# SJLeo/GCC

Hardware: AMD Instinct MI355X
Metric: training images/sec at 256x256 (pix2pix GCC) (higher is better)
Workload: dtype bf16; 1 GPU; Pix2Pix cityscapes 256x256 GCC distill+darts iteration (optimize_parameters + optimizer_netD_arch), student ngf32 / masked PatchGAN ndf128, teacher ngf64 / ndf128, filter_cfgs=None (no pretrained checkpoint to prune); batch_per_gpu=16, global_batch=16, image=256x256, parallelism=dp1, dropout=on (counter RNG; the oracle / golden iterations run --no_dropout)

## Files before the change

### gcc_amd/_lib.py

```python
import ctypes as C
import os

_HERE = os.path.dirname(os.path.abspath(__file__))
LIB_PATH = os.environ.get('GCC_HIP_LIB') or os.path.join(_HERE, 'libgcc_hip.so')

ACT_NONE, ACT_LRELU, ACT_RELU, ACT_TANH = 0, 1, 2, 3
GCC_HIP_ABI = 605
WGRAD_GROUP_MAX = 32
CHANSUM_GROUP_MAX = 24
SPECTRAL_GROUP_MAX = 8
CHANSUM_SMALL_MAX_PIXELS = 16384


class GccError(RuntimeError):
    pass


class conv_plan_t(C.Structure):
    _fields_ = [(n, C.c_int) for n in ('tile_families', 'big_min', 'big_nk', 'pair', 'halo_hc', 'wgrad_wgs_big', 'wgrad_wgs')]


PLAN_FIELDS = tuple(n for n, _ in conv_plan_t._fields_)


# ... 206 lines not shown
    'gcc_conv_eval_ex_workspace': (_Z, [C.POINTER(conv_t), _I]),
    'gcc_conv_eval_ex_route': (_I, [C.POINTER(conv_t), _I, _Z]),
    'gcc_conv_eval_f32': (_I, [C.POINTER(conv_t), _P, _P, _P, C.POINTER(eval_f32_epilogue_t), _P]),
    'gcc_conv_eval_f32_route': (_I, [C.POINTER(conv_t), _I]),
    'gcc_conv_eval_f32_kp': (_I, [_I, _I, _I]),
    'gcc_conv_eval_f32_ex': (_I, [C.POINTER(conv_t), _I, _I, _P, _P, _P, C.POINTER(eval_f32_epilogue_t), _P]),
    'gcc_conv_eval_f32_ex_route': (_I, [C.POINTER(conv_t), _I, _I, _I]),
    'gcc_conv_eval_f32_act': (_I, [C.POINTER(conv_t), _I, _I, _P, _P, _P, C.POINTER(eval_f32_act_epilogue_t), _P]),
    'gcc_conv_eval_f32_act_route': (_I, [C.POINTER(conv_t), _I, _I, _I, _I]),
    'gcc_conv_eval_f32_unet': (_I, [C.POINTER(conv_t), _I, _P, _P, _P, C.POINTER(eval_f32_unet_epilogue_t), _P]),
    'gcc_conv_eval_f32_unet_route': (_I, [C.POINTER(conv_t), _I]),
    'gcc_conv_eval_f32_unet_kp': (_I, [_I, _I]),
    'gcc_conv_eval_f32_resnet': (_I, [C.POINTER(conv_t), _I, _P, _P, _P, C.POINTER(eval_f32_resnet_epilogue_t), _P]),
    'gcc_conv_eval_f32_resnet_route': (_I, [C.POINTER(conv_t), _I]),
    'gcc_conv_eval_f32_resnet_kp': (_I, [_I, _I, _I]),
    'gcc_dwconv3x3_reflect_f32': (_I, [_P, _I, _P, _I, _P, _P, _I, _I, _I, _I, _P, _Z, _P]),
    'gcc_inorm_f32_workspace': (_Z, [_I, _I, C.c_longlong]),
    'gcc_inorm_stats_f32': (_I, [_P, _I, _I, _I, _I, _I, _P, _Z, _P]),
    'gcc_inorm_apply_f32': (_I, [_P, _I, _P, _I, _P, _I, _I, _I, _I, _I, _I, _F, _P, _Z, _P]),
    'gcc_nhwc_f32_to_nchw_f32': (_I, [_P, _P, _I, _I, _I, _I, _I, _I, _P]),
    'gcc_nchw_f32_to_nhwc_f32': (_I, [_P, _P, _I, _I, _I, _I, _I, _I, _I, _P]),
    'gcc_image_to_u8': (_I, [_P, _I, _I, _Z, _P, _P]),
    'gcc_image_to_u8_f32': (_I, [_P, _I, _I, _Z, _P, _P]),
    'gcc_dw_inorm_fwd': (_I, [C.POINTER(dw_inorm_t), _P]),
    'gcc_dw_inorm_route': (_I, [C.POINTER(dw_inorm_t)]),
    'gcc_dw_inorm_plan': (_I, [C.POINTER(dw_inorm_t), _I]),
    'gcc_conv_bn_act': (_I, [C.POINTER(conv_t), _I, _P, _P, _P, C.POINTER(bn_t), C.POINTER(bnact_t), _P, _I, _I, _P, _I, _I, _P, _Z, _P]),
    'gcc_conv_bn_act_plan': (_I, [C.POINTER(conv_t), _I, C.POINTER(bn_t), _I]),
    'gcc_bnact_bwd_workspace': (_Z, [_I, _Z]),
    'gcc_bnact_bwd': (_I, [C.POINTER(bnact_bwd_t), _P, _I, _I, _P, _I, _I, _P, _I, _I, _P, _I, _I, _P, _I, _I,
                           _I, _Z, _P, _Z, _P]),
    'gcc_bnact_bwd_ex': (_I, [C.POINTER(bnact_bwd_t), _I, _F, _P, _I, _I, _P, _I, _I, _P, _I, _I, _P, _I, _I, _P,
                              _I, _I, _I, _Z, _P, _Z, _P]),
    'gcc_channel_sum': (_I, [_P, _I, _I, _I, _Z, _P, _I, _P, _Z, _P]),
    'gcc_channel_sum_workspace': (_Z, [_I, _Z]),
    'gcc_channel_sum_group': (_I, [C.POINTER(chansum_item_t), _I, _P]),
    'gcc_gate_mask': (_I, [_P, _F, _P, _I, _P]),
    'gcc_gan_loss': (_I, [_I, _I, _I, _P, _I, _I, _Z, _F, _P, _I, _P, _P, _Z, _P]),
    'gcc_gan_loss_ex': (_I, [_I, _I, _I, _P, _I, _I, _Z, _P, _P, _F, _P, _I, _P]),
    'gcc_arch_coeffs': (_I, [_P, _P, _P, _P, _F, _P, _P, _P, _P]),
    'gcc_spectral_workspace': (_Z, [_I, _I, _I]),
    'gcc_spectral_power_iteration': (_I, [_P, _P, _P, _I, _I, _I, _P, _P, _P, _P, _Z, _P]),
    'gcc_spectral_power_iteration_pack': (_I, [_P, _P, _P, _I, _I, _I, _P, _P, _P, _P, _P, _Z, _P]),
    'gcc_spectral_group_workspace': (_Z, [C.POINTER(sn_item_t), _I]),
    'gcc_spectral_power_iteration_pack_group': (_I, [C.POINTER(sn_item_t), _I, _P, _Z, _P]),
    'gcc_spectral_eval_coeffs_workspace': (_Z, [C.POINTER(sn_eval_item_t), _I]),
    'gcc_spectral_eval_coeffs_group': (_I, [C.POINTER(sn_eval_item_t), _I, _P, _Z, _P]),
    'gcc_spectral_grad': (_I, [_P, _P, _P, _P, _P, _P, _I, _I, _I, _P, _P, _P, _P, _Z, _P]),
    'gcc_resample_u8': (_I, [_P, _I, _I, _Z, _P, _I, _I, _P, _P, _I, _P, _P, _I, _P, _P]),
    'gcc_crop_flip_normalize': (_I, [_P, _I, _I, _Z, _I, _I, _I, _I, _I, _P, _P, _I, _P]),
    'gcc_crop_convert': (_I, [_P, _I, _I, _Z, _I, _I, _I, _I, _I, _I, _P, _P, _P, _P, _I, _P]),
    'gcc_seg_input': (_I, [_P, _I, _I, _I, _I, _I, _I, _P, _P, _P, _P]),
    'gcc_miou_score': (_I, [_P, _I, _I, _I, _I, _P, _I, _I, _P, _P, _I, _P, _P, _I, _P, _P, _P]),
    'gcc_phase_regroup': (_I, [_P, _I, _I, _I, _P, _I, _I, _I, _I, _I, _I, _I, _P]),
    'gcc_relu_bf16': (_I, [_P, _I, _I, _I, _Z, _P]),
    'gcc_seg_head': (_I, [_P, _I, _I, _I, _I, _I, _I, _P, _P, _I, _P, _P, _P, _P]),
    'gcc_seg_head_f32': (_I, [_P, _I, _I, _I, _I, _I, _I, _P, _P, _I, _P, _P, _P, _P]),
    'gcc_fid_resize': (_I, [_P, _I, _I, _I, _P, _I, _I, _I, _I, _P]),
    'gcc_pool3x3': (_I, [_I, _P, _I, _I, _P, _I, _I, _I, _I, _I, _I, _P]),
    'gcc_border_copy': (_I, [_P, _I, _I, _P, _I, _I, _I, _I, _I, _I, _I, _I, _P]),
    'gcc_global_avgpool': (_I, [_P, _I, _I, _I, _I, _I, _I, _P, _P]),
    'gcc_fid_resize_f32': (_I, [_P, _I, _I, _I, _P, _I, _I, _I, _I, _P]),
    'gcc_pool3x3_f32': (_I, [_I, _P, _I, _I, _P, _I, _I, _I, _I, _I, _I, _P]),
    'gcc_global_avgpool_f32': (_I, [_P, _I, _I, _I, _I, _I, _I, _P, _P]),
    'gcc_argmax_channels': (_I, [_P, _I, _I, _Z, _P, _P]),
    'gcc_confusion_hist': (_I, [_P, _P, _Z, _I, _P, _P]),
    'gcc_psnr_workspace': (_Z, []),
# ... 80 lines not shown
```

### gcc_amd/csrc/norm_act.hip

```cpp
#include "common.hpp"
#include <stdlib.h>
#include <algorithm>
#include <mutex>
#include <unordered_map>

namespace {

struct Layout {
    int CH;
    int CHP;
    int sh;
    int PPB;
};
static bool make_layout(int C, Layout* L, int V = 8) {
    L->CH = ((C + 7) / 8) * (8 / V);
    if (L->CH > 256) return false;
    L->CHP = 1; L->sh = 0;
    while (L->CHP < L->CH) { L->CHP <<= 1; L->sh++; }
    L->PPB = 256 / L->CHP;
    return true;
}
static int stream_blocks(size_t pixels, const Layout& L, int sweeps_per_block) {
    constexpr size_t MAX_BLOCKS = 2048;
    size_t b = (pixels + (size_t)L.PPB * sweeps_per_block - 1) / ((size_t)L.PPB * sweeps_per_block);
// ... 156 lines not shown
        if (yg) *(i32x4*)(yg + pix * a.ldy + a.yoff + c0) = pack8(o1);
        if (y2g) *(i32x4*)(y2g + pix * a.ldy2 + a.y2off + c0) = pack8(o2);
    };
    const size_t step = (size_t)gridDim.x * a.L.PPB;
    const i32x4 z4 = {0, 0, 0, 0};
    for (size_t pix = (size_t)blockIdx.x * a.L.PPB + pl; pix < a.pixels; pix += 2 * step) {
        const size_t p1 = pix + step;
        const bool has1 = p1 < a.pixels;
        const i32x4 r0 = *(const i32x4*)(xg + pix * a.ldx + a.xoff + c0);
        const i32x4 r1 = has1 ? *(const i32x4*)(xg + p1 * a.ldx + a.xoff + c0) : z4;
        const i32x4 q0 = rg ? *(const i32x4*)(rg + pix * a.ldres + c0) : z4;
        const i32x4 q1 = (rg && has1) ? *(const i32x4*)(rg + p1 * a.ldres + c0) : z4;
        one(pix, r0, q0);
        if (has1) one(p1, r1, q1);
    }
}

struct BwdArgs {
    gcc_bnact_bwd_t p;
    const bf16_t* x; int ldx, xoff;
    const bf16_t* y; int ldy, yoff;
    const bf16_t* g1; int ldg1, g1off;
    const bf16_t* g2; int ldg2, g2off;
    bf16_t* dx; int lddx, dxoff;
    int C, C8; size_t pixels; Layout L;
    float* partial;
    float* totals;
    int in_act;
    float in_slope;
    int groups;
    int nblocks;
    unsigned* tickets;
    double* grp;
};

__device__ __forceinline__ BwdArgs group_view(const BwdArgs& a0) {
    BwdArgs a = a0;
    if (a0.groups > 1) {
        const size_t g = blockIdx.y;
        a.x += g * a0.pixels * a0.ldx;
        if (a.y) a.y += g * a0.pixels * a0.ldy;
        a.g1 += g * a0.pixels * a0.ldg1;
        if (a.g2) a.g2 += g * a0.pixels * a0.ldg2;
        a.dx += g * a0.pixels * a0.lddx;
        if (a.p.mean) a.p.mean = (const float*)a.p.mean + g * a0.C;
        if (a.p.rstd) a.p.rstd = (const float*)a.p.rstd + g * a0.C;
        a.partial += g * (size_t)a0.nblocks * 3 * a0.C8;
        a.totals += g * 3 * (size_t)a0.C8;
    }
    return a;
}

__device__ __forceinline__ void bwd_channel_finalize(const BwdArgs& a, int c, const double (&t)[3]) {
    if (c < a.C) {
        if (a.p.dbeta) a.p.dbeta[c] += (float)t[0];
        if (a.p.dgamma) a.p.dgamma[c] += (float)t[1];
        if (a.p.dalpha) a.p.dalpha[c] += (float)t[2];
    }
    float A = 0.f, B = 0.f, K = 0.f;
    if (c < a.C && a.p.bn && !a.p.bn_eval) {
        const float inv = 1.f / (float)a.pixels;
        const float rs = a.p.rstd[c], mu = a.p.mean[c];
        const float gr = (a.p.gamma ? a.p.gamma[c] : 1.f) * rs;
        const float k0 = (float)t[0] * inv, k1 = (float)t[1] * inv;
        A = gr; B = -gr * rs * k1; K = -gr * k0 + gr * rs * k1 * mu;
    }
// ... 27 lines not shown
        for (int r = 0; r < FIN_GROUP; r++)
            if (r < nr) sum += (double)v[r];
        __hip_atomic_store(a.grp + (size_t)g * W + idx, sum, __ATOMIC_RELAXED, __HIP_MEMORY_SCOPE_AGENT);
    }
    asm volatile("s_waitcnt vmcnt(0)" ::: "memory");
    __syncthreads();
    if (tid == 0) sh[0] = (int)__hip_atomic_fetch_add((gu32*)a.tickets + G, 1u, __ATOMIC_RELAXED, __HIP_MEMORY_SCOPE_AGENT);
    __syncthreads();
    const bool last = sh[0] == G - 1;
    __syncthreads();
    if (!last) return;
    for (int c = tid; c < a.C8; c += NT) {
        double t[3] = {0.0, 0.0, 0.0};
        for (int q0 = 0; q0 < G; q0 += 8) {
            i32x2 v[8][3];
#pragma unroll
            for (int u = 0; u < 8; u++) {
                const int q = q0 + u < G ? q0 + u : G - 1;
#pragma unroll
                for (int k = 0; k < 3; k++) v[u][k] = __builtin_amdgcn_raw_buffer_load_b64(rs_gr, (q * W + k * a.C8 + c) * 8, 0, 16);
            }
#pragma unroll
            for (int u = 0; u < 8; u++)
                if (q0 + u < G) {
#pragma unroll
                    for (int k = 0; k < 3; k++) t[k] += __builtin_bit_cast(double, v[u][k]);
                }
        }
        bwd_channel_finalize(a, c, t);
    }
    for (int i = tid; i <= G; i += NT) __hip_atomic_store((gu32*)a.tickets + i, 0u, __ATOMIC_RELAXED, __HIP_MEMORY_SCOPE_AGENT);
}

template <bool GATE, bool DROP, int V, int NTH>
__global__ __launch_bounds__(NTH) void bnact_bwd_reduce_kernel(const BwdArgs a0) {
    __shared__ float red[NTH][V + 1];
    const BwdArgs a = group_view(a0);
    const int ch = threadIdx.x & (a.L.CHP - 1);
    const int pl = threadIdx.x >> a.L.sh;
    const int c0 = ch * V;
    const bool active = ch < a.L.CH;
    const bool NOY = !a.y && a.p.bn;
    float mu[V], rs[V], sc[V], sf[V], gm[GATE ? V : 1];
    float s0[V], s1[V], s2[GATE ? V : 1];
#pragma unroll
    for (int j = 0; j < V; j++) {
        const int c = c0 + j;
        const bool v = active && c < a.C;
        mu[j] = (v && a.p.bn) ? a.p.mean[c] : 0.f;
        rs[j] = (v && a.p.bn) ? a.p.rstd[c] : (v ? 1.f : 0.f);
        if (GATE || DROP || NOY) {
            const float g = (v && a.p.bn && a.p.gamma) ? a.p.gamma[c] : 1.f;
            const float b = (v && a.p.bn && a.p.beta) ? a.p.beta[c] : 0.f;
            sc[j] = g * rs[j];
            sf[j] = b - mu[j] * sc[j];
        } else { sc[j] = 1.f; sf[j] = 0.f; }
        if constexpr (GATE) { gm[j] = v ? (a.p.gate ? a.p.gate[c] : 1.f) : 0.f; s2[j] = 0.f; }
        s0[j] = s1[j] = 0.f;
    }
    const float keep_scale = a.p.drop_p > 0.f ? 1.f / (1.f - a.p.drop_p) : 1.f;
    const float evs = (a.p.bn && a.p.bn_eval) ? 1.f : 0.f;
    if (active) {
        typedef typename RawVec<V>::type Raw;
        const size_t pstep = (size_t)gridDim.x * a.L.PPB;
        size_t pix = (size_t)blockIdx.x * a.L.PPB + pl;
        Raw rx = {}, ry = {}, rg1 = {}, rg2 = {};
        if (pix < a.pixels) {
            rx = ldraw<V>(a.x + pix * a.ldx + a.xoff + c0);
            if (a.y) ry = ldraw<V>(a.y + pix * a.ldy + a.yoff + c0);
            rg1 = ldraw<V>(a.g1 + pix * a.ldg1 + a.g1off + c0);
            if (a.g2) rg2 = ldraw<V>(a.g2 + pix * a.ldg2 + a.g2off + c0);
        }
        for (; pix < a.pixels; pix += pstep) {
            float xv[V], yv[V], g1v[V], g2v[V], dz[V];
            unraw(rx, xv); unraw(rg1, g1v);
            if (a.y) unraw(ry, yv);
            if (a.g2) unraw(rg2, g2v);
            const size_t nx = pix + pstep;
            if (nx < a.pixels) {
                rx = ldraw<V>(a.x + nx * a.ldx + a.xoff + c0);
                if (a.y) ry = ldraw<V>(a.y + nx * a.ldy + a.yoff + c0);
                rg1 = ldraw<V>(a.g1 + nx * a.ldg1 + a.g1off + c0);
                if (a.g2) rg2 = ldraw<V>(a.g2 + nx * a.ldg2 + a.g2off + c0);
            }
            float df[V], zd[V], g[V];
#pragma unroll
            for (int j = 0; j < V; j++) {
                df[j] = 1.f;
                if constexpr (DROP) {
                    const float u = rng_uniform(a.p.seed, pix * (size_t)a.C + c0 + j);
                    df[j] = u >= a.p.drop_p ? keep_scale : 0.f;
                }
                zd[j] = 0.f;
                if constexpr (GATE || DROP) zd[j] = (xv[j] * sc[j] + sf[j]) * df[j];
            }
            if constexpr (GATE) {
                if (!a.p.gate_after_act) {
                    float yo[V];
                    if (a.y) {
#pragma unroll
                        for (int j = 0; j < V; j++) yo[j] = yv[j];
                    } else {
                        float t[V];
#pragma unroll
                        for (int j = 0; j < V; j++) t[j] = zd[j] * gm[j];
                        apply_actN<V>(t, yo, a.p.act, a.p.slope);
                    }
#pragma unroll
                    for (int j = 0; j < V; j++) g[j] = g1v[j] * act_grad_from_out(yo[j], a.p.act, a.p.slope);
                    if (a.g2) {
#pragma unroll
                        for (int j = 0; j < V; j++) g[j] += g2v[j] * act_grad_from_out(yo[j], a.p.act2, a.p.slope);
                    }
#pragma unroll
                    for (int j = 0; j < V; j++) { s2[j] += g[j] * zd[j]; g[j] *= gm[j]; }
                } else {
// ... 1845 lines not shown
    if (b < 512) {
        const size_t lane_pixels = (size_t)L.PPB / 2 > 0 ? (size_t)L.PPB / 2 : 1;
        size_t sweeps = (pixels + lane_pixels * 512 - 1) / (lane_pixels * 512);
        if (sweeps < 2) sweeps = 2;
        if (sweeps > 16) sweeps = 16;
        b = (pixels + lane_pixels * sweeps - 1) / (lane_pixels * sweeps);
    }
    if (b < 1) b = 1;
    if (b > MAX_BLOCKS) b = MAX_BLOCKS;
    return (int)b;
}

constexpr size_t BWD_TICKET_BYTES = 4096;
extern "C" size_t gcc_bnact_bwd_workspace(int C, size_t pixels) {
    Layout L;
    if (C <= 0 || !make_layout(C, &L)) return 0;
    const int C8 = (C + 7) & ~7;
    const size_t blocks = (size_t)bwd_blocks(pixels, L);
    return BWD_TICKET_BYTES + (blocks + 1) * 3 * C8 * sizeof(float) + 64 + ((blocks + FIN_GROUP - 1) / FIN_GROUP) * 3 * C8 * sizeof(double);
}

extern "C" int gcc_bnact_bwd_ex(const gcc_bnact_bwd_t* p, int in_act, float in_slope, const void* x, int ldx, int xoff,
                                const void* y, int ldy, int yoff, const void* g1, int ldg1, int g1off, const void* g2,
                                int ldg2, int g2off, void* dx, int lddx, int dxoff, int C, size_t pixels, void* ws,
                                size_t ws_bytes, gcc_stream_t stream) {
    GCC_ENTER();
    if (!p || !x || !g1 || !dx || !ws || C <= 0 || pixels == 0) return GCC_ERR_BAD_ARG;
    if (!aligned8(ldx, xoff) || !aligned8(ldg1, g1off) || !aligned8(lddx, dxoff)) return GCC_ERR_BAD_ARG;
    if ((y && !aligned8(ldy, yoff)) || (g2 && !aligned8(ldg2, g2off))) return GCC_ERR_BAD_ARG;
    if (p->bn && (!p->mean || !p->rstd)) return GCC_ERR_BAD_ARG;
    const int groups = p->groups > 1 ? p->groups : 1;
    if (ws_bytes < gcc_bnact_bwd_workspace(C, pixels) * groups) return GCC_ERR_WORKSPACE;
    if (groups > 1 && (p->dgamma || p->dbeta || p->dalpha)) return GCC_ERR_UNSUPPORTED;
    BwdArgs a;
    a.p = *p;
    a.x = (const bf16_t*)x; a.ldx = ldx; a.xoff = xoff;
    a.y = (const bf16_t*)y; a.ldy = ldy; a.yoff = yoff;
    a.g1 = (const bf16_t*)g1; a.ldg1 = ldg1; a.g1off = g1off;
    a.g2 = (const bf16_t*)g2; a.ldg2 = ldg2; a.g2off = g2off;
    a.dx = (bf16_t*)dx; a.lddx = lddx; a.dxoff = dxoff;
    a.C = C; a.C8 = (C + 7) & ~7; a.pixels = pixels;
    a.in_act = in_act; a.in_slope = in_slope;
    if (!make_layout(C, &a.L)) return GCC_ERR_UNSUPPORTED;
    const int blocks = bwd_blocks(pixels, a.L);
    a.groups = groups; a.nblocks = blocks;
    a.partial = (float*)((char*)ws + BWD_TICKET_BYTES);
    a.totals = a.partial + (size_t)groups * blocks * 3 * a.C8;
    a.tickets = nullptr; a.grp = nullptr;
    const int G = (blocks + FIN_GROUP - 1) / FIN_GROUP;
    if ((p->flags & 1) && groups == 1 && (size_t)(G + 1) * 4 <= BWD_TICKET_BYTES) {
        a.tickets = (unsigned*)ws;
        a.grp = (double*)(((uintptr_t)(a.totals + (size_t)3 * a.C8) + 63) & ~(uintptr_t)63);
    }
    hipStream_t st = (hipStream_t)stream;
    const bool gate = p->gate != nullptr || p->dalpha != nullptr || p->gate_after_act;
    const bool drop = p->drop_p > 0.f;
    if (!p->bn && !gate && !drop && !p->dgamma && !p->dbeta && groups == 1 && gcc_opt(GCC_OPT_BN_BWD_SMALL)) {
        hipLaunchKernelGGL(act_bwd_kernel, dim3(stream_blocks(pixels, a.L, 4)), dim3(256), 0, st, a);
        GCC_CHECK_LAUNCH();
        return GCC_OK;
    }
    if (p->bn && !p->bn_eval && !gate && groups == 1 && pixels <= SMALL_MAX_PIXELS && gcc_opt(GCC_OPT_BN_BWD_SMALL)) {
        if (drop) hipLaunchKernelGGL(bnact_bwd_small_kernel<true>, dim3(a.C8 / 8), dim3(SMALL_NT), 0, st, a);
        else hipLaunchKernelGGL(bnact_bwd_small_kernel<false>, dim3(a.C8 / 8), dim3(SMALL_NT), 0, st, a);
        GCC_CHECK_LAUNCH();
        return GCC_OK;
    }
    {
        BwdArgs r = a;
        if (!make_layout(C, &r.L, 4)) return GCC_ERR_UNSUPPORTED;
        if (r.L.CHP > REDUCE_NT) return GCC_ERR_UNSUPPORTED;
        r.L.PPB = REDUCE_NT / r.L.CHP;
#define GCC_LAUNCH_REDUCE(G, D) \
        hipLaunchKernelGGL((bnact_bwd_reduce_kernel<G, D, 4, REDUCE_NT>), dim3(blocks, groups), dim3(REDUCE_NT), 0, st, r)
        if (gate && drop) GCC_LAUNCH_REDUCE(true, true);
        else if (gate) GCC_LAUNCH_REDUCE(true, false);
        else if (drop) GCC_LAUNCH_REDUCE(false, true);
        else GCC_LAUNCH_REDUCE(false, false);
#undef GCC_LAUNCH_REDUCE
    }
    GCC_CHECK_LAUNCH();
    if (!a.tickets) {
        hipLaunchKernelGGL(bnact_bwd_finalize_kernel, dim3((a.C8 + 31) / 32, groups), dim3(1024), 0, st, a, blocks);
        GCC_CHECK_LAUNCH();
    }
    if (p->bn && !p->bn_eval) {
        hipLaunchKernelGGL(bnact_bwd_apply_kernel, dim3(stream_blocks(pixels, a.L, 2), groups), dim3(256), 0, st, a);
        GCC_CHECK_LAUNCH();
    }
    return GCC_OK;
}

extern "C" int gcc_bnact_bwd(const gcc_bnact_bwd_t* p, const void* x, int ldx, int xoff, const void* y, int ldy, int yoff,
                             const void* g1, int ldg1, int g1off, const void* g2, int ldg2, int g2off, void* dx, int lddx,
                             int dxoff, int C, size_t pixels, void* ws, size_t ws_bytes, gcc_stream_t stream) {
    GCC_ENTER();
    return gcc_bnact_bwd_ex(p, GCC_ACT_NONE, 0.f, x, ldx, xoff, y, ldy, yoff, g1, ldg1, g1off, g2, ldg2, g2off, dx, lddx,
                            dxoff, C, pixels, ws, ws_bytes, stream);
}

extern "C" size_t gcc_channel_sum_workspace(int C, size_t pixels) {
    Layout L;
    if (C <= 0 || !make_layout(C, &L)) return 0;
    return (size_t)bwd_blocks(pixels, L) * ((C + 7) & ~7) * sizeof(float);
}

extern "C" int gcc_channel_sum(const void* x, int ld, int off, int C, size_t pixels, float* out, int accumulate,
                               void* ws, size_t ws_bytes, gcc_stream_t stream) {
    GCC_ENTER();
    if (!x || !out || !ws || C <= 0 || pixels == 0 || !aligned8(ld, off)) return GCC_ERR_BAD_ARG;
    if (ws_bytes < gcc_channel_sum_workspace(C, pixels)) return GCC_ERR_WORKSPACE;
    SumArgs a;
    a.x = (const bf16_t*)x; a.ld = ld; a.off = off; a.C = C; a.C8 = (C + 7) & ~7; a.pixels = pixels;
    a.partial = (float*)ws;
    if (!make_layout(C, &a.L)) return GCC_ERR_UNSUPPORTED;
    const int blocks = bwd_blocks(pixels, a.L);
    hipStream_t st = (hipStream_t)stream;
    if (pixels <= SUM_SMALL_MAX_PIXELS && gcc_opt(GCC_OPT_BN_BWD_SMALL)) {
        hipLaunchKernelGGL(channel_sum_small_kernel, dim3(a.C8 / 8), dim3(SUM_SMALL_NT), 0, st, a, out, accumulate);
        GCC_CHECK_LAUNCH();
        return GCC_OK;
    }
    hipLaunchKernelGGL(channel_sum_kernel, dim3(blocks), dim3(256), 0, st, a);
    GCC_CHECK_LAUNCH();
    hipLaunchKernelGGL(channel_sum_finalize_kernel, dim3((C + 31) / 32), dim3(1024), 0, st, (const float*)ws, blocks, C,
                       a.C8, out, accumulate);
    GCC_CHECK_LAUNCH();
    return GCC_OK;
}

extern "C" int gcc_channel_sum_group(const gcc_chansum_item_t* items, int n, gcc_stream_t stream) {
    GCC_ENTER();
    if (!items || n < 1 || n > GCC_CHANSUM_GROUP_MAX) return GCC_ERR_BAD_ARG;
// ... 44 lines not shown
```

### gcc_amd/engine.py

```python

import ctypes

import torch
import torch.nn as nn

from . import _lib, ops
from .ops import ACT_LRELU, ACT_NONE, ACT_RELU, ACT_TANH

LRELU = 0.2
OVERLAP_WGRAD = True


def overlap_wgrad_default(world):
    return world <= 1
WGRAD_GROUP_MAX_UNITS = 20000


class FlatParams:

    def __init__(self, params, device, layout=None):
        self.params = [p for p in params]
        if layout is None:
            layout = [self.params]
        placed = [p for seg in layout for p in seg]
# ... 884 lines not shown
                    _, stats = self.conv[li].forward(src, c.c[li], want_stats=True,
                                                     bn=ops.bn_desc(self.bn[li].bn, c.st[li], n, self.device, running=False))
                    c.deferred.append((li, stats, n))
                elif train:
                    self.conv[li].forward(src, c.c[li], want_stats=True, bn=self.bn[li].desc(c.st[li], n, self.device))
                else:
                    _, stats = self.conv[li].forward(src, c.c[li], want_stats=True)
                    self.bn[li].finalize(stats, n, c.st[li], train)
                ops.bnact_fwd(c.c[li], c.y[li], scale=c.st[li].scale, shift=c.st[li].shift, gate=self.mask[li], act=ACT_LRELU)
            src = c.y[li]
        self.conv[L - 1].forward(src, c.pred)
        c.train = train
        return c.pred

    def apply_deferred_running(self, c):
        for li, stats, n in getattr(c, 'deferred', []):
            stats.record_stream(ops.current_stream())
            self.bn[li].finalize(stats, n, c.st[li], True)
        c.deferred = []

    def backward(self, c, has_pred_grad=True, g_feat=None, wgrad=True, agrad=False, need_dx=True, gslot=0, dalpha=None):
        L = self.L
        G = self._gbufs(c.N, c.H, c.W, gslot)
        assert gslot == 0 or not wgrad

        def agrad_of(li):
            if not agrad or self.gate[li] is None:
                return None
            return dalpha[li] if dalpha is not None else self.gate[li].alpha.grad
        if g_feat is None:
            g_feat = [None, None]
        feat_of = {1: g_feat[0], 3: g_feat[1]}
        wg = WgradCollector(self, c)
        if has_pred_grad:
            if wgrad:
                wg.add(self.conv[L - 1], c.y[L - 2], G.layer[L - 1], seg=0)
            self.conv[L - 1].backward_data(G.layer[L - 1], G.layer[L - 2])
        for li in range(L - 2, 0, -1):
            g1, g2 = G.layer[li], feat_of.get(li)
            if li == L - 2 and not has_pred_grad:
                assert g2 is not None, 'nothing to back-propagate'
                g1, g2 = g2, None
            gate = self.gate[li]
            if self.inorm[li]:
                if g2 is None and c.hs[li][0] * c.hs[li][1] <= ops.INORM_FUSED_MAX_HW:
                    ops.inorm_bwd(c.c[li], c.y[li], g1, G.layer[li], c.st[li], act=ACT_LRELU)
                else:
                    ops.bnact_bwd(c.c[li], c.y[li], g1, G.layer[li], g2=g2, bn=c.st[li], act=ACT_LRELU, act2=ACT_LRELU, groups=c.N)
            else:
                bn = self.bn[li].bn
                ops.bnact_bwd(c.c[li], None, g1, G.layer[li], g2=g2, bn=c.st[li], gamma=bn.weight.data, beta=bn.bias.data,
                              gate=self.mask[li], act=ACT_LRELU, act2=ACT_LRELU, dgamma=bn.weight.grad if wgrad else None,
                              dbeta=bn.bias.grad if wgrad else None,
                              dalpha=agrad_of(li))
            src = c.g0 if li == 1 else c.y[li - 1]
            if wgrad:
                wg.add(self.conv[li], src, G.layer[li], seg=L - 1 - li)
            self.conv[li].backward_data(G.layer[li], G.layer[li - 1])
        gate = self.gate[0]
        b0 = self.conv[0].bias
        ops.bnact_bwd(c.a0, None, G.layer[0], G.layer[0], gate=self.mask[0], gate_after_act=True, in_act=ACT_LRELU,
                      dalpha=agrad_of(0),
                      dbeta=b0.grad if (wgrad and b0 is not None) else None)
        if wgrad:
            wg.add(self.conv[0], c.x_in, G.layer[0], seg=L - 1, bias_done=True)
        dx = None
        if need_dx:
            self.conv[0].backward_data(G.layer[0], G.x_in)
            dx = G.x_in
        wg.flush('all')
        ops.SideStream.get(self.device).join()
        return dx


class DWOp:

    def __init__(self, conv):
# ... 1655 lines not shown
```

### gcc_amd/ops.py

```python
import ctypes as C
import os
import threading

import torch

from . import _lib
from ._lib import ACT_LRELU, ACT_NONE, ACT_RELU, ACT_TANH, check

_ws_cache = {}


class _Profile:

    def __init__(self):
        self.active = False
        self.spans_only = False
        self.records = []
        self.streaming = os.environ.get('GCC_PROFILE_STREAMING') == '1'

    def start(self, steps=None):
        self.records = []
        self.spans = []
        self.tag = None
        self.active = True
# ... 1497 lines not shown
            and (g2 is not None or drop_p > 0.0 or (y is None and act != ACT_NONE) or pixels <= BN_BWD_GRID_MIN_PIXELS)
            and (BN_BWD_GRID_EX >= 2 or pixels <= BN_BWD_GRID_EX_MAX_PIXELS)):
        ws = inorm_workspace(x.device)
        rc = lib().gcc_bn_bwd_one_launch_ex(xp, ldx, yp, ldy, g1p, ldg1, g2p, ldg2, dxp, lddx, Cc, pixels, act, act2, slope, drop_p, seed,
                                            bn.mean.data_ptr(), bn.rstd.data_ptr(), bn.scale.data_ptr(), bn.shift.data_ptr(),
                                            _p(gamma), _p(dgamma), _p(dbeta), ws.data_ptr(), ws.numel(), stream())
        if rc == 0:
            return
        if rc != -2:
            check(rc, 'gcc_bn_bwd_one_launch_ex')
    if (BN_BWD_GRID and bn is not None and not bn_eval and g2 is None and gate is None and not gate_after_act and drop_p == 0.0
            and dalpha is None and in_act == ACT_NONE and act2 == ACT_NONE and groups <= 1 and (y is not None or act == ACT_NONE)
            and pixels > BN_BWD_GRID_MIN_PIXELS and pixels * ceil8(Cc) * 2 <= BN_BWD_GRID_MAX_BYTES and not PROFILE.active):
        ws = inorm_workspace(x.device)
        rc = lib().gcc_bn_bwd_one_launch(xp, ldx, yp, ldy, g1p, ldg1, dxp, lddx, Cc, pixels, act, slope, bn.mean.data_ptr(),
                                         bn.rstd.data_ptr(), _p(gamma), _p(dgamma), _p(dbeta), ws.data_ptr(), ws.numel(), stream())
        if rc == 0:
            return
        if rc != -2:
            check(rc, 'gcc_bn_bwd_one_launch')
    p = _lib.bnact_bwd_t(1 if bn is not None else 0, int(bn_eval), _p(bn.mean) if bn is not None else None,
                         _p(bn.rstd) if bn is not None else None, _p(gamma), _p(beta), _p(gate), int(gate_after_act),
                         act, slope, act2, drop_p, seed, _p(dgamma), _p(dbeta), _p(dalpha), groups, 1 if BN_BWD_TAIL else 0)
    need = lib().gcc_bnact_bwd_workspace(Cc, pixels) * max(1, groups)
    ws = zeroed_workspace(x.device, 'bnbwd', need) if BN_BWD_TAIL else workspace(need, x.device, 'bnbwd')
    e0 = PROFILE.begin() if (PROFILE.active and PROFILE.streaming) else None
    check(lib().gcc_bnact_bwd_ex(C.byref(p), in_act, slope, xp, ldx, 0, yp, ldy, 0, g1p, ldg1, 0, g2p, ldg2, 0, dxp, lddx,
                                 0, Cc, pixels, ws.data_ptr(), ws.numel(), stream()), 'gcc_bnact_bwd')
    if e0 is not None:
        PROFILE.end('bnact_bwd (bytes)', float(N * H * W * ceil8(Cc)) * (14.0 if (bn is not None and not bn_eval) else 6.0), e0,
                    shape=('bnbwd', N, Cc, H, W, 'bn' if bn is not None else 'act', 'gate' if gate is not None else ''))


def channel_sum(x, out, accumulate=False):
    xp, N, Cc, H, W, ld = geom(x)
    need = lib().gcc_channel_sum_workspace(Cc, N * H * W)
    ws = workspace(need, x.device, 'chansum')
    check(lib().gcc_channel_sum(xp, ld, 0, Cc, N * H * W, out.data_ptr(), int(accumulate), ws.data_ptr(), ws.numel(),
                                stream()), 'gcc_channel_sum')


def channel_sum_group(pairs, accumulate=True):
    small = []
    for x, out in pairs:
        xp, N, Cc, H, W, ld = geom(x)
        if N * H * W <= _lib.CHANSUM_SMALL_MAX_PIXELS:
            small.append((xp, ld, Cc, N * H * W, out.data_ptr()))
        else:
            channel_sum(x, out, accumulate=accumulate)
    for i in range(0, len(small), _lib.CHANSUM_GROUP_MAX):
        part = small[i:i + _lib.CHANSUM_GROUP_MAX]
        items = (_lib.chansum_item_t * len(part))()
        for it, (xp, ld, Cc, px, op) in zip(items, part):
            it.x, it.ld, it.off, it.C, it.pixels, it.out, it.accumulate = xp, ld, 0, Cc, px, op, int(accumulate)
        check(lib().gcc_channel_sum_group(items, len(part), stream()), 'gcc_channel_sum_group')


def gate_mask(alpha, tau, mask):
    check(lib().gcc_gate_mask(alpha.data_ptr(), float(tau), mask.data_ptr(), alpha.numel(), stream()), 'gcc_gate_mask')


GAN_MODES = {'hinge': 0, 'lsgan': 1, 'vanilla': 2, 'wgangp': 3}


def gan_loss(mode, pred, target_is_real, for_discriminator, loss, dpred=None, grad_weight=1.0, weight_dev=None,
             dpred_accumulate=False):
# ... 302 lines not shown
```

### include/gcc_hip.h

```cpp
#ifndef GCC_HIP_H
#define GCC_HIP_H

#include <stddef.h>
#include <stdint.h>

#ifdef __cplusplus
extern "C" {
#endif

typedef void* gcc_stream_t;

enum {
    GCC_OK = 0,
    GCC_ERR_BAD_ARG = -1,
    GCC_ERR_UNSUPPORTED = -2,
    GCC_ERR_WORKSPACE = -3,
    GCC_ERR_LAUNCH = -4
};

enum { GCC_ACT_NONE = 0, GCC_ACT_LRELU = 1, GCC_ACT_RELU = 2, GCC_ACT_TANH = 3 };

#define GCC_HIP_ABI 605

const char* gcc_strerror(int code);
// ... 295 lines not shown
                             gcc_stream_t stream);

int gcc_image_to_u8(const void* x, int ld, int off, size_t pixels, void* out, gcc_stream_t stream);
int gcc_image_to_u8_f32(const float* x, int ld, int off, size_t pixels, void* out, gcc_stream_t stream);

typedef struct {
    int bn;
    int bn_eval;
    const float* mean;
    const float* rstd;
    const float* gamma;
    const float* beta;
    const float* gate;
    int gate_after_act;
    int act; float slope;
    int act2;
    float drop_p; uint64_t seed;
    float* dgamma; float* dbeta; float* dalpha;
    int groups;
    int flags;
} gcc_bnact_bwd_t;

size_t gcc_bnact_bwd_workspace(int C, size_t pixels);
int gcc_bnact_bwd(const gcc_bnact_bwd_t* p, const void* x, int ldx, int xoff, const void* y, int ldy, int yoff,
                  const void* g1, int ldg1, int g1off, const void* g2, int ldg2, int g2off,
                  void* dx, int lddx, int dxoff, int C, size_t pixels, void* ws, size_t ws_bytes,
                  gcc_stream_t stream);

int gcc_bnact_bwd_ex(const gcc_bnact_bwd_t* p, int in_act, float in_slope, const void* x, int ldx, int xoff,
                     const void* y, int ldy, int yoff, const void* g1, int ldg1, int g1off, const void* g2,
                     int ldg2, int g2off, void* dx, int lddx, int dxoff, int C, size_t pixels, void* ws,
                     size_t ws_bytes, gcc_stream_t stream);

int gcc_reflect_pad(const void* src, int lds, void* dst, int ldd, int N, int H, int W, int C, int pad, int backward,
                    gcc_stream_t stream);
int gcc_dwconv3x3_reflect(int mode, const void* x, int ldx, const void* dy, int lddy, void* out, int ldo, const float* w,
                          const float* bias, int N, int H, int W, int C, gcc_stream_t stream);
size_t gcc_dwconv3x3_wgrad_workspace(int N, int H, int W, int C);
int gcc_dwconv3x3_reflect_wgrad(const void* x, int ldx, const void* dy, int lddy, float* dw, float* dbias, int N, int H,
                                int W, int C, void* ws, size_t ws_bytes, gcc_stream_t stream);

int gcc_channel_sum(const void* x, int ld, int off, int C, size_t pixels, float* out, int accumulate,
                    void* ws, size_t ws_bytes, gcc_stream_t stream);
size_t gcc_channel_sum_workspace(int C, size_t pixels);
#define GCC_CHANSUM_GROUP_MAX 24
#define GCC_CHANSUM_SMALL_MAX_PIXELS 16384
typedef struct {
    const void* x;
    int ld, off, C;
    size_t pixels;
    float* out;
    int accumulate;
} gcc_chansum_item_t;
int gcc_channel_sum_group(const gcc_chansum_item_t* items, int n, gcc_stream_t stream);

int gcc_gate_mask(const float* alpha, float tau, float* mask, int C, gcc_stream_t stream);

int gcc_gan_loss(int mode, int target_is_real, int for_discriminator, const void* pred, int ld, int off,
                 size_t pixels, float weight, float* loss, int accumulate, void* dpred,
                 void* ws, size_t ws_bytes, gcc_stream_t stream);
int gcc_gan_loss_ex(int mode, int target_is_real, int for_discriminator, const void* pred, int ld, int off,
                    size_t pixels, float* loss, void* dpred, float grad_weight, const float* grad_weight_dev,
                    int dpred_accumulate, gcc_stream_t stream);
int gcc_arch_coeffs(const float* Lfr, const float* Lf, const float* Lr, const float* dT, float real_fake_weight,
                    float* loss, float* c_fr, float* c_f, gcc_stream_t stream);
int gcc_l1_loss(const void* a, int lda, int aoff, const void* b, int ldb, int boff, int C, size_t pixels,
// ... 193 lines not shown
```

Baseline: 1076 images/s.

## Fuse PatchGAN head conv data-grad into BN/activation backward reduce kernel

Adds a gcc_bnact_bwd_head path that computes the final 4x4 Co=1 discriminator conv's input gradient on the fly inside the BN/activation backward reduce kernel, using bf16 dot2 over 16 taps, instead of running a separate backward_data conv and reading its output back. Two variants are provided: per-thread 16-tap loads, and a lane-cooperative load with DPP/readlane broadcast. This removes a kernel launch and a full-resolution gradient write and read. The cost is extra per-pixel index math, added register pressure (with a waves_per_eu hint), and rounding through bf16 to match the unfused path.

```diff
diff --git a/gcc_amd/_lib.py b/gcc_amd/_lib.py
--- a/gcc_amd/_lib.py
+++ b/gcc_amd/_lib.py
@@ -262,7 +262,9 @@
                            _I, _Z, _P, _Z, _P]),
     'gcc_bnact_bwd_ex': (_I, [C.POINTER(bnact_bwd_t), _I, _F, _P, _I, _I, _P, _I, _I, _P, _I, _I, _P, _I, _I, _P,
                               _I, _I, _I, _Z, _P, _Z, _P]),
-    'gcc_channel_sum': (_I, [_P, _I, _I, _I, _Z, _P, _I, _P, _Z, _P]),
+    'gcc_bnact_bwd_head': (_I, [C.POINTER(bnact_bwd_t), _I, _F, _P, _I, _I, _P, _I, _I, _P, _I, _I, _P, _I, _I, _I, _I, _I,
+                                _P, _I, _I, _P, _I, _I, _I, _I, _I, _I, _P, _Z, _P]),
+    'gcc_channel_sum':(_I, [_P, _I, _I, _I, _Z, _P, _I, _P, _Z, _P]),
     'gcc_channel_sum_workspace': (_Z, [_I, _Z]),
     'gcc_channel_sum_group': (_I, [C.POINTER(chansum_item_t), _I, _P]),
     'gcc_gate_mask': (_I, [_P, _F, _P, _I, _P]),
diff --git a/gcc_amd/csrc/norm_act.hip b/gcc_amd/csrc/norm_act.hip
--- a/gcc_amd/csrc/norm_act.hip
+++ b/gcc_amd/csrc/norm_act.hip
@@ -212,6 +212,10 @@
     int nblocks;
     unsigned* tickets;
     double* grp;
+    const bf16_t* dp; int lddp, dpoff;
+    const bf16_t* hw; int ldhw;
+    int Hm, Wm;
+    FastDiv dHW, dW;
 };
 
 __device__ __forceinline__ BwdArgs group_view(const BwdArgs& a0) {
@@ -305,8 +309,69 @@
     for (int i = tid; i <= G; i += NT) __hip_atomic_store((gu32*)a.tickets + i, 0u, __ATOMIC_RELAXED, __HIP_MEMORY_SCOPE_AGENT);
 }
 
-template <bool GATE, bool DROP, int V, int NTH>
-__global__ __launch_bounds__(NTH) void bnact_bwd_reduce_kernel(const BwdArgs a0) {
+struct HeadPix { int n, y, x; };
+__device__ __forceinline__ HeadPix head_pixel(const BwdArgs& a, int pix) {
+    HeadPix h;
+    h.n = fdiv(pix, a.dHW);
+    const int r = pix - h.n * (a.Hm * a.Wm);
+    h.y = fdiv(r, a.dW);
+    h.x = r - h.y * a.Wm;
+    return h;
+}
+__device__ __forceinline__ void head_load(const BwdArgs& a, int pix, uint32_t (&q)[16]) {
+    typedef __attribute__((address_space(4))) const uint32_t cu32;
+    const HeadPix h = head_pixel(a, pix);
+    const int Hp = a.Hm - 1, Wp = a.Wm - 1;
+#pragma unroll
+    for (int t = 0; t < 16; t++) {
+        const int py = h.y + 1 - (t >> 2), px = h.x + 1 - (t & 3);
+        const bool in = (unsigned)py < (unsigned)Hp && (unsigned)px < (unsigned)Wp;
+        const size_t e = (in ? ((size_t)(h.n * Hp + py) * Wp + px) * a.lddp : (size_t)0) + a.dpoff;
+        q[t] = ((cu32*)a.dp)[e >> 1];
+    }
+}
+__device__ __forceinline__ void head_taps(const BwdArgs& a, int pix, const uint32_t (&q)[16], uint32_t (&dp)[8]) {
+    const HeadPix h = head_pixel(a, pix);
+    const int Hp = a.Hm - 1, Wp = a.Wm - 1;
+    const bool hi = a.dpoff & 1;
+#pragma unroll
+    for (int u = 0; u < 8; u++) {
+        uint32_t v[2];
+#pragma unroll
+        for (int s = 0; s < 2; s++) {
+            const int t = 2 * u + s;
+            const int py = h.y + 1 - (t >> 2), px = h.x + 1 - (t & 3);
+            const bool in = (unsigned)py < (unsigned)Hp && (unsigned)px < (unsigned)Wp;
+            v[s] = in ? (hi ? q[t] >> 16 : q[t] & 0xffffu) : 0u;
+        }
+        dp[u] = v[0] | (v[1] << 16);
+    }
+}
+__device__ __forceinline__ uint32_t head_lane_load(const BwdArgs& a, int pix, uint32_t* m) {
+    typedef __attribute__((address_space(4))) const uint32_t cu32;
+    const HeadPix h = head_pixel(a, pix);
+    const int Hp = a.Hm - 1, Wp = a.Wm - 1;
+    const int t = threadIdx.x & 15;
+    const int py = h.y + 1 - (t >> 2), px = h.x + 1 - (t & 3);
+    const bool in = (unsigned)py < (unsigned)Hp && (unsigned)px < (unsigned)Wp;
+    const uint32_t e = (in ? (uint32_t)((h.n * Hp + py) * Wp + px) * (uint32_t)a.lddp : 0u) + (uint32_t)a.dpoff;
+    *m = in ? ((a.dpoff & 1) ? 0xffff0000u : 0xffffu) : 0u;
+    return ((cu32*)a.dp)[e >> 1];
+}
+__device__ __forceinline__ void head_lane_taps(const BwdArgs& a, uint32_t q, uint32_t m, uint32_t (&dp)[8]) {
+    const uint32_t v = (q & m) >> ((a.dpoff & 1) * 16);
+    const uint32_t nb = (uint32_t)__builtin_amdgcn_mov_dpp((int)v, 0xB1, 0xf, 0xf, true);
+    const uint32_t pr = v | (nb << 16);
+#pragma unroll
+    for (int u = 0; u < 8; u++) dp[u] = (uint32_t)__builtin_amdgcn_readlane((int)pr, 2 * u);
+}
+__device__ __forceinline__ float dot2_bf16(uint32_t a, uint32_t b, float acc) {
+    typedef __attribute__((ext_vector_type(2))) __bf16 bf16x2;
+    return __builtin_amdgcn_fdot2_f32_bf16(__builtin_bit_cast(bf16x2, a), __builtin_bit_cast(bf16x2, b), acc, false);
+}
+
+template <bool GATE, bool DROP, int V, int NTH, int HEAD = 0>
+__global__ __launch_bounds__(NTH) __attribute__((amdgpu_waves_per_eu(HEAD ? 4 : 1))) void bnact_bwd_reduce_kernel(const BwdArgs a0) {
     __shared__ float red[NTH][V + 1];
     const BwdArgs a = group_view(a0);
     const int ch = threadIdx.x & (a.L.CHP - 1);
@@ -338,23 +403,57 @@
         const size_t pstep = (size_t)gridDim.x * a.L.PPB;
         size_t pix = (size_t)blockIdx.x * a.L.PPB + pl;
         Raw rx = {}, ry = {}, rg1 = {}, rg2 = {};
+        uint32_t hw[HEAD ? 8 : 1][V];
+        uint32_t hq[HEAD == 1 ? 16 : 1], hm = 0;
+        if constexpr (HEAD) {
+            static_assert(!HEAD || V == 4, "the head's weights are paired for 4 channels per thread");
+#pragma unroll
+            for (int u = 0; u < 8; u++) {
+                const i32x2 w0 = ldraw<4>(a.hw + (size_t)(2 * u) * a.ldhw + c0), w1 = ldraw<4>(a.hw + (size_t)(2 * u + 1) * a.ldhw + c0);
+#pragma unroll
+                for (int h = 0; h < 2; h++) {
+                    hw[u][2 * h] = ((uint32_t)w0[h] & 0xffffu) | ((uint32_t)w1[h] << 16);
+                    hw[u][2 * h + 1] = ((uint32_t)w0[h] >> 16) | ((uint32_t)w1[h] & 0xffff0000u);
+                }
+            }
+        }
         if (pix < a.pixels) {
             rx = ldraw<V>(a.x + pix * a.ldx + a.xoff + c0);
             if (a.y) ry = ldraw<V>(a.y + pix * a.ldy + a.yoff + c0);
-            rg1 = ldraw<V>(a.g1 + pix * a.ldg1 + a.g1off + c0);
+            if constexpr (HEAD == 1) head_load(a, (int)pix, hq);
+            else if constexpr (HEAD == 2) hq[0] = head_lane_load(a, __builtin_amdgcn_readfirstlane((int)pix), &hm);
+            else rg1 = ldraw<V>(a.g1 + pix * a.ldg1 + a.g1off + c0);
             if (a.g2) rg2 = ldraw<V>(a.g2 + pix * a.ldg2 + a.g2off + c0);
         }
         for (; pix < a.pixels; pix += pstep) {
             float xv[V], yv[V], g1v[V], g2v[V], dz[V];
-            unraw(rx, xv); unraw(rg1, g1v);
+            unraw(rx, xv);
+            uint32_t dp[8];
+            if constexpr (HEAD == 1) head_taps(a, (int)pix, hq, dp);
+            else if constexpr (HEAD == 2) head_lane_taps(a, hq[0], hm, dp);
+            else unraw(rg1, g1v);
             if (a.y) unraw(ry, yv);
             if (a.g2) unraw(rg2, g2v);
             const size_t nx = pix + pstep;
             if (nx < a.pixels) {
                 rx = ldraw<V>(a.x + nx * a.ldx + a.xoff + c0);
                 if (a.y) ry = ldraw<V>(a.y + nx * a.ldy + a.yoff + c0);
-                rg1 = ldraw<V>(a.g1 + nx * a.ldg1 + a.g1off + c0);
+                if constexpr (HEAD == 1) head_load(a, (int)nx, hq);
+                else if constexpr (HEAD == 2) hq[0] = head_lane_load(a, __builtin_amdgcn_readfirstlane((int)nx), &hm);
+                else rg1 = ldraw<V>(a.g1 + nx * a.ldg1 + a.g1off + c0);
                 if (a.g2) rg2 = ldraw<V>(a.g2 + nx * a.ldg2 + a.g2off + c0);
+            }
+            if constexpr (HEAD) {
+                float acc[V];
+#pragma unroll
+                for (int j = 0; j < V; j++) acc[j] = 0.f;
+#pragma unroll
+                for (int u = 0; u < 8; u++) {
+#pragma unroll
+                    for (int j = 0; j < V; j++) acc[j] = dot2_bf16(hw[u][j], dp[u], acc[j]);
+                }
+#pragma unroll
+                for (int j = 0; j < V; j++) g1v[j] = bf2f(f2bf(acc[j]));
             }
             float df[V], zd[V], g[V];
 #pragma unroll
@@ -2266,7 +2365,7 @@
     const int groups = p->groups > 1 ? p->groups : 1;
     if (ws_bytes < gcc_bnact_bwd_workspace(C, pixels) * groups) return GCC_ERR_WORKSPACE;
     if (groups > 1 && (p->dgamma || p->dbeta || p->dalpha)) return GCC_ERR_UNSUPPORTED;
-    BwdArgs a;
+    BwdArgs a = {};
     a.p = *p;
     a.x = (const bf16_t*)x; a.ldx = ldx; a.xoff = xoff;
     a.y = (const bf16_t*)y; a.ldy = ldy; a.yoff = yoff;
@@ -2333,6 +2432,68 @@
                             dxoff, C, pixels, ws, ws_bytes, stream);
 }
 
+extern "C" int gcc_bnact_bwd_head(const gcc_bnact_bwd_t* p, int in_act, float in_slope, const void* x, int ldx, int xoff,
+                                  const void* y, int ldy, int yoff, const void* dpred, int lddp, int dpoff, const void* w,
+                                  int ldw, int k, int stride, int pad, int Co, const void* g2, int ldg2, int g2off, void* dx,
+                                  int lddx, int dxoff, int C, int N, int H, int W, void* ws, size_t ws_bytes,
+                                  gcc_stream_t stream) {
+    GCC_ENTER();
+    if (!p || !x || !dpred || !w || !dx || !ws || C <= 0 || N <= 0 || H <= 0 || W <= 0) return GCC_ERR_BAD_ARG;
+    if (!aligned8(ldx, xoff) || !aligned8(lddx, dxoff) || (g2 && !aligned8(ldg2, g2off))) return GCC_ERR_BAD_ARG;
+    if ((lddp & 7) || dpoff < 0 || dpoff >= lddp || ((uintptr_t)dpred & 3)) return GCC_ERR_BAD_ARG;
+    const int C8 = (C + 7) & ~7;
+    if ((ldw & 7) || ldw < C8 || ((uintptr_t)w & 15)) return GCC_ERR_BAD_ARG;
+    if (p->bn && (!p->mean || !p->rstd)) return GCC_ERR_BAD_ARG;
+    if (p->groups > 1 || (p->bn && p->bn_eval) || p->drop_p > 0.f || y) return GCC_ERR_UNSUPPORTED;
+    if (k != 4 || stride != 1 || pad != 1 || Co != 1 || H < 2 || W < 2) return GCC_ERR_UNSUPPORTED;
+    if ((size_t)N * H * W >= (size_t)1 << 31 || (size_t)N * (H - 1) * (W - 1) * lddp >= (size_t)1 << 31) return GCC_ERR_UNSUPPORTED;
+    const size_t pixels = (size_t)N * H * W;
+    BwdArgs a = {};
+    Layout L4;
+    if (!make_layout(C, &a.L) || !make_layout(C, &L4, 4) || L4.CHP > REDUCE_NT) return GCC_ERR_UNSUPPORTED;
+    if (ws_bytes < gcc_bnact_bwd_workspace(C, pixels)) return GCC_ERR_WORKSPACE;
+    a.p = *p;
+    a.x = (const bf16_t*)x; a.ldx = ldx; a.xoff = xoff;
+    a.g2 = (const bf16_t*)g2; a.ldg2 = ldg2; a.g2off = g2off;
+    a.dx = (bf16_t*)dx; a.lddx = lddx; a.dxoff = dxoff;
+    a.C = C; a.C8 = C8; a.pixels = pixels;
+    a.in_act = in_act; a.in_slope = in_slope;
+    a.dp = (const bf16_t*)dpred; a.lddp = lddp; a.dpoff = dpoff;
+    a.hw = (const bf16_t*)w; a.ldhw = ldw;
+    a.Hm = H; a.Wm = W; a.dHW = make_fastdiv(H * W); a.dW = make_fastdiv(W);
+    const int blocks = bwd_blocks(pixels, a.L);
+    a.groups = 1; a.nblocks = blocks;
+    a.partial = (float*)((char*)ws + BWD_TICKET_BYTES);
+    a.totals = a.partial + (size_t)blocks * 3 * a.C8;
+    const int G = (blocks + FIN_GROUP - 1) / FIN_GROUP;
+    if ((p->flags & 1) && (size_t)(G + 1) * 4 <= BWD_TICKET_BYTES) {
+        a.tickets = (unsigned*)ws;
+        a.grp = (double*)(((uintptr_t)(a.totals + (size_t)3 * a.C8) + 63) & ~(uintptr_t)63);
+    }
+    hipStream_t st = (hipStream_t)stream;
+    const bool gate = p->gate != nullptr || p->dalpha != nullptr || p->gate_after_act;
+    {
+        BwdArgs r = a;
+        r.L = L4;
+        r.L.PPB = REDUCE_NT / r.L.CHP;
+#define GCC_LAUNCH_HEAD(G, U) \
+        hipLaunchKernelGGL((bnact_bwd_reduce_kernel<G, false, 4, REDUCE_NT, U>), dim3(blocks), dim3(REDUCE_NT), 0, st, r)
+        if (r.L.CHP >= 64 && ((r.L.CH & 63) == 0 || (r.L.CH & 63) >= 16)) { if (gate) GCC_LAUNCH_HEAD(true, 2); else GCC_LAUNCH_HEAD(false, 2); }
+        else { if (gate) GCC_LAUNCH_HEAD(true, 1); else GCC_LAUNCH_HEAD(false, 1); }
+#undef GCC_LAUNCH_HEAD
+    }
+    GCC_CHECK_LAUNCH();
+    if (!a.tickets) {
+        hipLaunchKernelGGL(bnact_bwd_finalize_kernel, dim3((a.C8 + 31) / 32), dim3(1024), 0, st, a, blocks);
+        GCC_CHECK_LAUNCH();
+    }
+    if (p->bn) {
+        hipLaunchKernelGGL(bnact_bwd_apply_kernel, dim3(stream_blocks(pixels, a.L, 2)), dim3(256), 0, st, a);
+        GCC_CHECK_LAUNCH();
+    }
+    return GCC_OK;
+}
+
 extern "C" size_t gcc_channel_sum_workspace(int C, size_t pixels) {
     Layout L;
     if (C <= 0 || !make_layout(C, &L)) return 0;
diff --git a/gcc_amd/engine.py b/gcc_amd/engine.py
--- a/gcc_amd/engine.py
+++ b/gcc_amd/engine.py
@@ -940,17 +940,28 @@
             g_feat = [None, None]
         feat_of = {1: g_feat[0], 3: g_feat[1]}
         wg = WgradCollector(self, c)
+        head_done = False
         if has_pred_grad:
             if wgrad:
                 wg.add(self.conv[L - 1], c.y[L - 2], G.layer[L - 1], seg=0)
-            self.conv[L - 1].backward_data(G.layer[L - 1], G.layer[L - 2])
+            if L >= 3 and self.bn[L - 2] is not None:
+                bn, hc = self.bn[L - 2].bn, self.conv[L - 1]
+                head_done = ops.bnact_bwd_head(c.c[L - 2], G.layer[L - 1], hc.w, hc.k, hc.stride, hc.pad, G.layer[L - 2],
+                                               g2=feat_of.get(L - 2), bn=c.st[L - 2], gamma=bn.weight.data, beta=bn.bias.data,
+                                               gate=self.mask[L - 2], act=ACT_LRELU, act2=ACT_LRELU,
+                                               dgamma=bn.weight.grad if wgrad else None, dbeta=bn.bias.grad if wgrad else None,
+                                               dalpha=agrad_of(L - 2))
+            if not head_done:
+                self.conv[L - 1].backward_data(G.layer[L - 1], G.layer[L - 2])
         for li in range(L - 2, 0, -1):
             g1, g2 = G.layer[li], feat_of.get(li)
             if li == L - 2 and not has_pred_grad:
                 assert g2 is not None, 'nothing to back-propagate'
                 g1, g2 = g2, None
             gate = self.gate[li]
-            if self.inorm[li]:
+            if li == L - 2 and head_done:
+                pass
+            elif self.inorm[li]:
                 if g2 is None and c.hs[li][0] * c.hs[li][1] <= ops.INORM_FUSED_MAX_HW:
                     ops.inorm_bwd(c.c[li], c.y[li], g1, G.layer[li], c.st[li], act=ACT_LRELU)
                 else:
diff --git a/gcc_amd/ops.py b/gcc_amd/ops.py
--- a/gcc_amd/ops.py
+++ b/gcc_amd/ops.py
@@ -1553,6 +1553,37 @@
                     shape=('bnbwd', N, Cc, H, W, 'bn' if bn is not None else 'act', 'gate' if gate is not None else ''))
 
 
+BN_BWD_HEAD = True
+
+
+def bnact_bwd_head(x, dpred, w, k, stride, pad, dx, g2=None, bn=None, gamma=None, beta=None, gate=None, act=ACT_NONE, slope=0.2,
+                   act2=ACT_NONE, dgamma=None, dbeta=None, dalpha=None):
+    if not BN_BWD_HEAD or PROFILE.active or w.dim() != 3 or w.shape[1] != k * k:
+        return False
+    xp, N, Cc, H, W, ldx = geom(x)
+    pixels = N * H * W
+    if (gate is None and dalpha is None and pixels <= BN_BWD_GRID_MIN_PIXELS
+            and (BN_BWD_GRID_EX or lib().gcc_get_option(_lib.OPT_BN_BWD_SMALL))):
+        return False
+    dpp, _, Co, Hp, Wp, lddp = geom(dpred)
+    assert (Hp, Wp) == ((H + 2 * pad - k) // stride + 1, (W + 2 * pad - k) // stride + 1) and dpred.shape[0] == N
+    g2p, ldg2 = (None, 0)
+    if g2 is not None:
+        g2p, _, _, _, _, ldg2 = geom(g2)
+    dxp, _, _, _, _, lddx = geom(dx)
+    p = _lib.bnact_bwd_t(1 if bn is not None else 0, 0, _p(bn.mean) if bn is not None else None,
+                         _p(bn.rstd) if bn is not None else None, _p(gamma), _p(beta), _p(gate), 0, act, slope, act2, 0.0, 0,
+                         _p(dgamma), _p(dbeta), _p(dalpha), 1, 1 if BN_BWD_TAIL else 0)
+    need = lib().gcc_bnact_bwd_workspace(Cc, pixels)
+    ws = zeroed_workspace(x.device, 'bnbwd', need) if BN_BWD_TAIL else workspace(need, x.device, 'bnbwd')
+    rc = lib().gcc_bnact_bwd_head(C.byref(p), ACT_NONE, slope, xp, ldx, 0, None, 0, 0, dpp, lddp, 0, w.data_ptr(), w.shape[2], k, stride,
+                                  pad, Co, g2p, ldg2, 0, dxp, lddx, 0, Cc, N, H, W, ws.data_ptr(), ws.numel(), stream())
+    if rc == -2:
+        return False
+    check(rc, 'gcc_bnact_bwd_head')
+    return True
+
+
 def channel_sum(x, out, accumulate=False):
     xp, N, Cc, H, W, ld = geom(x)
     need = lib().gcc_channel_sum_workspace(Cc, N * H * W)
diff --git a/include/gcc_hip.h b/include/gcc_hip.h
--- a/include/gcc_hip.h
+++ b/include/gcc_hip.h
@@ -351,6 +351,11 @@
                      int ldg2, int g2off, void* dx, int lddx, int dxoff, int C, size_t pixels, void* ws,
                      size_t ws_bytes, gcc_stream_t stream);
 
+int gcc_bnact_bwd_head(const gcc_bnact_bwd_t* p, int in_act, float in_slope, const void* x, int ldx, int xoff,
+                       const void* y, int ldy, int yoff, const void* dpred, int lddp, int dpoff, const void* w, int ldw,
+                       int k, int stride, int pad, int Co, const void* g2, int ldg2, int g2off, void* dx, int lddx,
+                       int dxoff, int C, int N, int H, int W, void* ws, size_t ws_bytes, gcc_stream_t stream);
+
 int gcc_reflect_pad(const void* src, int lds, void* dst, int ldd, int N, int H, int W, int C, int pad, int backward,
                     gcc_stream_t stream);
 int gcc_dwconv3x3_reflect(int mode, const void* x, int ldx, const void* dy, int lddy, void* out, int ldo, const float* w,
```

Result: no change. 1084 images/s, median of 6 (+0.7%).
